# praisechan/Chameleon-RAG-Acceleration

Measured on AMD Instinct MI355X. Metric: queries/sec + recall@10, SIFT1M IVF-PQ (nlist=1024, M=16, nprobe=16), higher is better.
Workload: dtype f32; 1 GPU; IVF1024,PQ16x8 search, d=128, nb=1000000, nprobe=16, k=10, batch=1024 queries per GPU per step; parallelism=single GPU, global_batch=1024, inflight=2, key=nb1000000-d128-IVF1024-PQ16-np16-k10-B1024-w1-single-c200000

## Files before the change

chameleon-rag-acceleration_amd/csrc/ivfpq_index.cpp:

```cpp
#include <hip/hip_runtime.h>

#include <algorithm>
#include <cmath>
#include <cstdio>
#include <cstdlib>
#include <cstring>
#include <memory>
#include <mutex>
#include <stdexcept>
#include <string>
#include <vector>

#include "ivfpq.h"
#include "ivfpq_test.h"
#include "ivfpq_kernels.h"
#include "ivfpq_build.h"
#include "pq_flat.h"

using namespace chivf;

namespace {

thread_local std::string g_err;

// ... 32 lines not shown
  ~DevBuf() { release(); }
};

struct DeviceGuard {
  int prev = -1;
  explicit DeviceGuard(int dev) {
    HIPCHECK(hipGetDevice(&prev));
    if (prev != dev) HIPCHECK(hipSetDevice(dev));
  }
  ~DeviceGuard() {
    int cur = -1;
    if (hipGetDevice(&cur) == hipSuccess && cur != prev && prev >= 0) (void)hipSetDevice(prev);
  }
};

uint64_t splitmix(uint64_t* s) {
  uint64_t z = (*s += 0x9E3779B97F4A7C15ull);
  z = (z ^ (z >> 30)) * 0xBF58476D1CE4E5B9ull;
  z = (z ^ (z >> 27)) * 0x94D049BB133111EBull;
  return z ^ (z >> 31);
}

std::vector<int64_t> rand_perm_prefix(int64_t n, int64_t k, uint64_t seed) {
  std::vector<int64_t> p(n), out(k);
  for (int64_t i = 0; i < n; i++) p[i] = i;
  uint64_t s = seed;
  for (int64_t i = 0; i < k; i++) {
    int64_t j = i + (int64_t)(splitmix(&s) % (uint64_t)(n - i));
    std::swap(p[i], p[j]);
    out[i] = p[i];
  }
  return out;
}

void renorm_rows(float* x, int64_t n, int d) {
  for (int64_t i = 0; i < n; i++) {
    float* xi = x + i * d;
    float nr = 0.f;
    for (int t = 0; t < d; t++) nr += xi[t] * xi[t];
    if (nr > 0.f) {
      const float inv = (float)(1.0 / (double)sqrtf(nr));
      for (int t = 0; t < d; t++) xi[t] *= inv;
    }
  }
}

void kmeans_update(const float* x, int64_t n, int d, int k, const int64_t* assign, float* cent) {
  std::vector<double> sum((size_t)k * d, 0.0);
  std::vector<int64_t> cnt(k, 0);
  for (int64_t i = 0; i < n; i++) {
    const int64_t c = assign[i];
    cnt[c]++;
    double* s = &sum[(size_t)c * d];
    const float* xi = x + i * d;
    for (int t = 0; t < d; t++) s[t] += (double)xi[t];
  }
  for (int c = 0; c < k; c++)
    if (cnt[c] > 0)
      for (int t = 0; t < d; t++) cent[(size_t)c * d + t] = (float)(sum[(size_t)c * d + t] / (double)cnt[c]);
  const float eps = 1.0f / 1024.0f;
  for (int c = 0; c < k; c++) {
    if (cnt[c] != 0) continue;
    int big = 0;
    for (int j = 1; j < k; j++)
      if (cnt[j] > cnt[big]) big = j;
    for (int t = 0; t < d; t++) {
      const float v = cent[(size_t)big * d + t];
      if (t % 2 == 0) {
        cent[(size_t)c * d + t] = v * (1.0f + eps);
        cent[(size_t)big * d + t] = v * (1.0f - eps);
      } else {
        cent[(size_t)c * d + t] = v * (1.0f - eps);
        cent[(size_t)big * d + t] = v * (1.0f + eps);
      }
    }
    cnt[c] = cnt[big] / 2;
    cnt[big] -= cnt[c];
  }
}

constexpr size_t kChunkBytes = size_t(256) << 20;
constexpr size_t kPartialBytes = size_t(2048) << 20;
constexpr int kSegmentedNlist = 8192;
constexpr int kInflightFreeCus = 16;

bool inflight_default() {
  const char* e = std::getenv("IVFPQ_INFLIGHT");
  return e && e[0] == '1';
}

}

struct ivfpq_index {
  int d = 0, nlist = 0, M = 0, nbits = 8, ksub = 256, metric = IVFPQ_METRIC_L2, device = 0;
  int nprobe = 1;
  int list_lo = 0, list_hi = 0;
  bool trained = false;
  std::vector<float> centroids, codebook;
  std::vector<std::vector<uint8_t>> lcodes;
  std::vector<std::vector<int64_t>> lids;
  int64_t ntotal = 0;
  int64_t next_id = 0;

  DevBuf d_cent, d_centT, d_cnorm, d_cb, d_T1, d_codes, d_ids, d_off, d_order;
  bool dirty = true;
  hipStream_t stream = nullptr;
  DevBuf w_x, w_xn, w_D, w_I, w_lno, w_codes, w_cent, w_cn;
  DevBuf h_D, h_I, h_Iq, h_Dq;
  DevBuf q_lists, q_ids, q_codes, a_off;
  int64_t q_n = 0, q_kept = 0, q_cap = 0;
  int64_t img_n = 0;
  bool host_stale = false;
  struct PreT3 {
    DevBuf buf;
    int64_t n = 0;
    uint64_t seq = 0;
    uint64_t freed_seq = 0;
    hipEvent_t ready = nullptr;
    hipStream_t ready_stream = nullptr;
    hipEvent_t freed = nullptr;
    hipStream_t freed_stream = nullptr;
    bool ready_pending = false, freed_pending = false;
  };
  static constexpr int kPreT3 = 3;
  PreT3 pre[kPreT3];
  uint64_t pre_seq = 0;
  struct Work {
    DevBuf w_dist, w_lists, w_dis0, w_T3, w_cand;
    DevBuf w_qn;
    DevBuf p_cnt, p_bucket, p_recs, p_hdr, p_part, p_N, p_pd0, p_done, p_tau, p_qmask, p_evlog;
    uint32_t epoch = 0;
    hipEvent_t done = nullptr;
    hipStream_t done_stream = nullptr;
    bool done_pending = false;
    uint64_t last_use = 0;
  };
  static constexpr int kSlots = 3;
  Work work[kSlots];
  int slot = 0;
  uint64_t uses = 0;
  bool inflight = inflight_default();
  int fault_inj = 0;
  std::vector<uint64_t> tau_seed;
  std::mutex mu;

  Work& W() { return work[slot]; }
  void begin_slot(hipStream_t s) {
    int pick = -1;
    for (int i = 0; i < kSlots && pick < 0; i++)
      if (work[i].done_pending && work[i].done_stream == s) pick = i;
    if (pick < 0) {
      pick = 0;
      for (int i = 1; i < kSlots; i++)
        if (work[i].last_use < work[pick].last_use) pick = i;
    }
    slot = pick;
    Work& w = work[slot];
    w.last_use = ++uses;
    if (w.done_pending && w.done_stream != s) {
      HIPCHECK(hipEventSynchronize(w.done));
      w.done_pending = false;
    }
    if (!inflight) order_after_all(s);
  }
  void order_after_all(hipStream_t s) {
    for (auto& w : work)
      if (w.done_pending && w.done_stream != s) HIPCHECK(hipStreamWaitEvent(s, w.done, 0));
  }
  void mark_done(hipStream_t s) {
    Work& w = W();
    HIPCHECK(hipEventRecord(w.done, s));
    w.done_stream = s;
    w.done_pending = true;
  }
  void quiesce() {
    for (auto& w : work) {
      if (w.done_pending) HIPCHECK(hipEventSynchronize(w.done));
      w.done_pending = false;
    }
  }

  ListPlan make_plan(int64_t nq, int np, int k, hipStream_t s, bool leave_free = false) {
    const int nloc = std::max(list_hi - list_lo, 1);
    Work& w = W();
    const int G = list_scan_group(M, k);
    ListPlan pl;
    pl.cap = (int)nq;
    pl.max_items = list_scan_max_items(nq * np, nloc, G);
    pl.grid = scan_lists_grid(M, k, leave_free ? kInflightFreeCus : 0);
    if (!w.p_cnt.p || w.p_cnt.bytes < sizeof(int32_t) * 2 * nloc) {
      w.p_cnt.ensure(sizeof(int32_t) * 2 * nloc);
      HIPCHECK(hipMemsetAsync(w.p_cnt.p, 0, w.p_cnt.bytes, s));
    }
    w.p_bucket.ensure(sizeof(int2) * 2 * (size_t)nloc * nq);
    w.p_recs.ensure(sizeof(int32_t) * 16 * (size_t)pl.max_items);
    if (!w.p_hdr.p) {
      w.p_hdr.ensure(sizeof(int32_t) * 16);
      HIPCHECK(hipMemsetAsync(w.p_hdr.p, 0, w.p_hdr.bytes, s));
    }
    pl.ks = part_stride(k);
    w.p_part.ensure(sizeof(uint4) * nq * np * 4 * pl.ks);
    w.p_N.ensure(sizeof(uint2) * nq * np * 4);
    w.p_pd0.ensure(sizeof(float) * nq * np);
    if (!w.p_evlog.p) {
      w.p_evlog.ensure(sizeof(uint32_t) * 8 * kEvLog);
      HIPCHECK(hipMemsetAsync(w.p_evlog.p, 0, w.p_evlog.bytes, s));
    }
    if (!w.p_done.p || w.p_done.bytes < sizeof(int32_t) * nq) {
      w.p_done.ensure(sizeof(int32_t) * nq);
      HIPCHECK(hipMemsetAsync(w.p_done.p, 0, w.p_done.bytes, s));
    }
    if (!w.p_tau.p || w.p_tau.bytes < sizeof(uint64_t) * nq) {
      w.p_tau.ensure(sizeof(uint64_t) * nq);
      HIPCHECK(hipMemsetAsync(w.p_tau.p, 0xff, w.p_tau.bytes, s));
    }
    if (++w.epoch >= 0xFFFFFFF0u) {
      if (w.done_pending) HIPCHECK(hipEventSynchronize(w.done));
      HIPCHECK(hipMemsetAsync(w.p_tau.p, 0xff, w.p_tau.bytes, s));
      w.epoch = 1;
    }
    if (!tau_seed.empty()) {
      std::vector<uint64_t> seed;
      seed.swap(tau_seed);
      require((int64_t)seed.size() == nq, "seeded bounds: one per query of the next batch (single-chunk searches)");
      for (auto& v : seed) v = ((uint64_t)(~w.epoch) << 32) | (uint32_t)v;
      HIPCHECK(hipMemcpyAsync(w.p_tau.p, seed.data(), sizeof(uint64_t) * nq, hipMemcpyHostToDevice, s));
      HIPCHECK(hipStreamSynchronize(s));
    }
    pl.qmw = (np + 63) / 64;
    w.p_qmask.ensure(sizeof(uint64_t) * nq * pl.qmw);
    pl.cnt = w.p_cnt.as<int32_t>();
    pl.bucket = w.p_bucket.as<int2>();
    pl.recs = w.p_recs.as<int32_t>();
    pl.hdr = w.p_hdr.as<int32_t>();
    pl.part = w.p_part.as<uint4>();
    pl.partN = w.p_N.as<uint2>();
    pl.pd0 = w.p_pd0.as<float>();
    pl.evlog = w.p_evlog.as<uint32_t>();
    pl.fault = fault_inj;
    pl.qdone = w.p_done.as<int32_t>();
    pl.tauq = w.p_tau.as<uint64_t>();
    pl.epoch = w.epoch;
    pl.err = w.p_hdr.as<int32_t>() + 15;
    pl.qmask = w.p_qmask.as<uint64_t>();
    pl.order = d_order.p ? d_order.as<int32_t>() : nullptr;
    pl.fused = scan_fused_plan(nloc, pl.max_items, M) ? 1 : 0;
    return pl;
  }

  enum Stage { ST_COARSE = 0, ST_TABLES = 1, ST_SCAN = 2, ST_LISTS = 3, ST_N = 4 };
  int timing = 0;
  struct Mark {
    int stage;
    hipEvent_t a, b;
  };
  std::vector<Mark> marks;
  std::vector<hipEvent_t> ev_pool;

  hipEvent_t take_event() {
    if (!ev_pool.empty()) {
      hipEvent_t e = ev_pool.back();
      ev_pool.pop_back();
      return e;
    }
    hipEvent_t e;
    HIPCHECK(hipEventCreate(&e));
    return e;
  }
  int mark_begin(int stage, hipStream_t s, bool record = true) {
    if (!timing || (timing == 2 && stage != ST_LISTS)) return -1;
    Mark m{stage, take_event(), take_event()};
    if (record) HIPCHECK(hipEventRecord(m.a, s));
    marks.push_back(m);
    return (int)marks.size() - 1;
  }
  void mark_end(int idx, hipStream_t s) {
    if (idx >= 0) HIPCHECK(hipEventRecord(marks[idx].b, s));
  }
  void collect_timing(double* ms, int64_t* cnt) {
    for (int i = 0; i < ST_N; i++) {
      ms[i] = 0.0;
      cnt[i] = 0;
    }
    for (auto& m : marks) {
      HIPCHECK(hipEventSynchronize(m.b));
      float t = 0.f;
      HIPCHECK(hipEventElapsedTime(&t, m.a, m.b));
      ms[m.stage] += t;
      cnt[m.stage] += 1;
      ev_pool.push_back(m.a);
      ev_pool.push_back(m.b);
    }
    marks.clear();
  }

  ~ivfpq_index() {
    for (auto& m : marks) {
      (void)hipEventDestroy(m.a);
      (void)hipEventDestroy(m.b);
    }
    for (auto e : ev_pool) (void)hipEventDestroy(e);
    for (auto& w : work)
      if (w.done) (void)hipEventDestroy(w.done);
    for (auto& p : pre) {
      if (p.ready) (void)hipEventDestroy(p.ready);
      if (p.freed) (void)hipEventDestroy(p.freed);
    }
    if (stream) (void)hipStreamDestroy(stream);
  }

  void init_stream() {
    if (!stream) HIPCHECK(hipStreamCreateWithFlags(&stream, hipStreamNonBlocking));
    for (auto& w : work)
      if (!w.done) HIPCHECK(hipEventCreateWithFlags(&w.done, hipEventDisableTiming));
    for (auto& p : pre) {
      if (!p.ready) HIPCHECK(hipEventCreateWithFlags(&p.ready, hipEventDisableTiming));
      if (!p.freed) HIPCHECK(hipEventCreateWithFlags(&p.freed, hipEventDisableTiming));
    }
  }

  void assign_top1(const float* x_host, int64_t n, int dd, const float* dc, const float* dcn, int nc,
                   int64_t* assign_host, const float* x_dev = nullptr, bool ip_assign = false) {
    const int64_t rows = std::max<int64_t>(1, std::min<int64_t>(n, kChunkBytes / ((size_t)nc * 4)));
    w_xn.ensure(sizeof(float) * rows);
    W().w_dist.ensure(sizeof(float) * rows * nc);
    w_D.ensure(sizeof(float) * rows);
    w_I.ensure(sizeof(int64_t) * rows);
    if (!x_dev) w_x.ensure(sizeof(float) * rows * dd);
    for (int64_t r0 = 0; r0 < n; r0 += rows) {
// ... 1580 lines not shown
```

chameleon-rag-acceleration_amd/csrc/ivfpq_kernels.h:

```cpp
#pragma once
#include <hip/hip_runtime.h>
#include <stdint.h>

namespace chivf {

constexpr int kMaxK = 1024;
constexpr int64_t kSentinelId = INT64_MAX;

void launch_row_norms(const float* x, int64_t n, int d, float* out, hipStream_t s);

void launch_l2_dist(const float* x, const float* xn, int64_t nx, const float* c, const float* cn, int nc, int d,
                    float* out, hipStream_t s, bool ip = false);

void launch_select_rows(const float* dist, int64_t nrows, int ncols, int n, float* out_val, int64_t* out_col,
                        hipStream_t s, bool neg = false);

struct ListPlan;

bool coarse_tiled_ok(int d, int64_t nq);
void launch_coarse_keys(const float* x, int64_t nq, int d, const float* centT, const float* cn, int nlist,
                        float* keys, hipStream_t s, bool ip, float* T3out = nullptr, const float* cb = nullptr,
                        int M = 0, float* xn_buf = nullptr, const float* xt = nullptr, int64_t nt = 0,
                        bool hoist = false);
void launch_coarse_select(const float* keys, int64_t nq, int nlist, int nprobe, float* out_dis, int64_t* out_list,
                          hipStream_t s, bool ip, const ListPlan* plan = nullptr, const int64_t* list_off = nullptr,
                          int lo = 0, int hi = 0, const float* x = nullptr, const float* cent = nullptr, int d = 0);

int coarse_segments(int64_t nq, int nlist, int d);
void launch_coarse_segmented(const float* x, int64_t nq, int d, const float* centT, const float* cn, int nlist,
                             int nprobe, uint64_t* cand, float* out_dis, int64_t* out_list, hipStream_t s, bool ip,
                             const ListPlan* plan = nullptr, const int64_t* list_off = nullptr, int lo = 0, int hi = 0,
                             const float* cent = nullptr);

void launch_linear_transform(const float* x, int64_t n, int d_in, const float* AT, const float* b, int d_out, float* y,
                             hipStream_t s);

void launch_ip_table(const float* x, int64_t n, int d, const float* codebook, int M, int ksub, float* out,
                     hipStream_t s);

void launch_precompute_T1(const float* cent, int nlist, int d, const float* codebook, int M, int ksub, float* T1,
                          hipStream_t s);

void launch_pq_encode(const float* x, int64_t n, int d, const float* cent, const int64_t* list_no,
                      const float* codebook, int M, int ksub, uint8_t* codes, hipStream_t s);

inline int part_stride(int k) { return k; }

constexpr int kHdrLog = 12;
constexpr int kHdrStale = 13;
constexpr int kHdrRepair = 14;
constexpr int kEvLog = 64;

struct ListPlan {
  int32_t* cnt;
  int2* bucket;
  int cap;
  int32_t* recs;
  int32_t* hdr;
  int max_items;
  uint4* part;
  uint2* partN;
  float* pd0;
  int32_t* qdone;
  uint64_t* tauq;
  uint32_t epoch;
  int32_t* err;
  uint64_t* qmask;
  int qmw = 1;
  uint32_t* evlog;
  int fault = 0;
  int grid;
  const int32_t* order = nullptr;
  int fused = 0;
  int ks = 0;
};

struct ScanArgs {
  const float* T1;
  const float* T3;
  const uint8_t* codes;
  const int64_t* ids;
  const int64_t* list_off;
  int64_t n_codes;
  const int64_t* probe_list;
  int64_t nq;
  int nprobe;
  int k;
  int M;
  int ip;
  int list_lo, list_hi;
  float* outD;
  int64_t* outI;
};

void launch_plan_count(const int64_t* lists, const float* Dq, const float* x, const float* cent, int64_t nq, int d,
                       int nprobe, const int64_t* list_off, int lo, int hi, bool ip, bool dedup, int k,
                       const ListPlan& pl, hipStream_t s);
void launch_plan_items(const ListPlan& pl, const int64_t* list_off, int lo, int hi, int G, hipStream_t s);
bool scan_fused_plan(int nloc, int max_items, int M);

int list_scan_group(int M, int k);
int list_scan_max_items(int64_t npairs, int nloc, int G);
int scan_lists_grid(int M, int k, int free_cus = 0);
bool scan_supported_M(int M);
void launch_scan_lists(const ScanArgs& a, const ListPlan& plan, hipStream_t s, hipEvent_t* ev_lists = nullptr);

void launch_merge_topk(int S, int64_t n, int k, const float* Din, const int64_t* Iin, float* Dout, int64_t* Iout,
                       hipStream_t s, bool ip = false);

}
```

chameleon-rag-acceleration_amd/csrc/ivfpq_kernels.hip:

```cpp
#include <float.h>
#include <stdint.h>

#include <algorithm>
#include <type_traits>

#include <hip/hip_runtime.h>

#include "ivfpq_kernels.h"
#include "ivfpq_diag.h"

namespace chivf {

namespace {

constexpr float kInf = __builtin_huge_valf();

enum { K_IP = 0, K_L2 = 1, K_NORM = 2 };

template <int KIND, class FX, class FY>
__device__ __forceinline__ float tree(FX fx, FY fy, int d) {
  float a8[8] = {0.f, 0.f, 0.f, 0.f, 0.f, 0.f, 0.f, 0.f};
  int i = 0;
  for (; i + 8 <= d; i += 8) {
#pragma unroll
// ... 2111 lines not shown
#pragma unroll
                for (int g = 0; g < G; g++) {
                  if ((mk[g] >> lane) & 1) {
                    const int sl = g * QG + qn[g] + __popcll(mk[g] & lanemask_lt);
                    qd[wave][sl] = dis[j][g];
                    qi[wave][sl] = i;
                  }
                  qn[g] += __popcll(mk[g]);
                  DIAG_ONLY(d_push += __popcll(mk[g]);)
                }
                if (loose) {
                  stop = j + 1;
                  want = true;
                  go = false;
                }
              }
            }
          }
        }
        if (stop >= tn) {
          pend = want;
          break;
        }
        drain();
        t = stop;
      }
      bool queued = false;
#pragma unroll
      for (int g = 0; g < G; g++) queued = queued || qn[g] > 0;
      DIAG_ONLY(const uint64_t tc0 = __builtin_amdgcn_s_memtime(); d_admit += tc0 - tb0;)
      if (pend || (last_sb && queued)) {
        drain();
      }
      DIAG_ONLY(asm volatile("" ::"v"(ROWK ? rk : tk[0].p[0])); d_fdrain += __builtin_amdgcn_s_memtime() - tc0;)
    }
    DIAG(2, __builtin_amdgcn_s_memtime());
    DIAG(4, n);
    DIAG(5, it.cnt | (it.kind << 8));
    DIAG(6, d_gather);
    DIAG(7, d_push | (d_drain << 32));
    DIAG(8, d_loose);
    DIAG(9, d_admit);
    DIAG(10, d_fdrain);

    if constexpr (ROWK) {
      const int rg = lane >> 4, re = lane & 15;
      int pr = it.pair[0];
#pragma unroll
      for (int g = 1; g < G; g++) pr = rg == g ? it.pair[g] : pr;
      const int64_t slot = (int64_t)pr * 4 + wave;
      if (rg < it.cnt && re < k && !(pl.fault > 0 && slot % pl.fault == 1)) {
        const bool empty = rk == kKcNone;
        pl.part[slot * pl.ks + re] =
            part_rec(empty ? FLT_MAX : kc_key(rk), part_tag(pl.epoch, slot) | xcc_tag(), empty ? -1 : it.beg + (int64_t)(uint32_t)rk);
      }
    } else {
#pragma unroll
      for (int g = 0; g < G; g++) {
        if (g >= it.cnt) continue;
        write_partial<R>(pl, tk[g], (int64_t)it.pair[g] * 4 + wave, k, it.beg, lane);
      }
    }
    if (nxt >= 0) {
      unpack(nrec);
      if constexpr (kEarly) issue();
    }
    DIAG(3, __builtin_amdgcn_s_memtime());
    it_no++;
    cur = nxt;
  }
}

#ifndef SCAN_LEAN
#define SCAN_LEAN 1
#endif
#ifndef SCAN_PREFETCH
#define SCAN_PREFETCH 0
#endif
constexpr bool kScanLean = SCAN_LEAN != 0;
constexpr bool kScanPrefetch = SCAN_PREFETCH != 0;
#ifndef SCAN_LEAN_JB
#define SCAN_LEAN_JB 6
#endif
constexpr int kLeanJB = SCAN_LEAN_JB;

__device__ __forceinline__ uint64_t pack_kc_bits(uint32_t b, uint32_t pos) {
  b = b == 0x80000000u ? 0u : b;
  const uint32_t o = (int32_t)b >= 0 ? (b ^ 0x80000000u) : ~b;
  return ((uint64_t)o << 32) | pos;
}
__device__ __forceinline__ uint64_t row_shr1_u64(uint64_t v) {
  const uint32_t lo = (uint32_t)__builtin_amdgcn_update_dpp((int)(uint32_t)v, (int)(uint32_t)v, 0x111, 0xf, 0xf, false);
  const uint32_t hi =
      (uint32_t)__builtin_amdgcn_update_dpp((int)(uint32_t)(v >> 32), (int)(uint32_t)(v >> 32), 0x111, 0xf, 0xf, false);
  return ((uint64_t)hi << 32) | lo;
}

template <int M, int JB>
__global__ __launch_bounds__(256, 2) void k_scan_lean(ScanArgs a, ListPlan pl) {
  constexpr int G = 4;
  constexpr int LUTN = M * 256;
  constexpr int NV = LUTN / 4 / 256;
  static_assert(NV <= 4 && JB % 2 == 0, "lean scan: M <= 16");
  __shared__ __attribute__((aligned(16))) float4 lut[LUTN];
  __shared__ int s_next;
  __shared__ int32_t s_wb[G];
  __shared__ int s_ws[8];
  __shared__ uint16_t s_ex[2][kFusedPlanLists + 1];
  __shared__ uint16_t s_ord[kFusedPlanLists];

  const int tid = threadIdx.x;
  const int lane = tid & 63;
  const int wave = __builtin_amdgcn_readfirstlane(tid >> 6);
  const int k = a.k;
  const int ip = a.ip;
  const int nloc = a.list_hi - a.list_lo;
  const float inv_np = 1.0f / (float)a.nprobe;
  const int rg = lane >> 4, re = lane & 15;
  const int2 nn = fused_plan_prefix(pl, nloc, G, s_ex[0], s_ex[1], s_ord, s_ws);
  const int n_items0 = nn.x, n_items = nn.x + nn.y;

  Item<G> it;
  auto unpack = [&](const Rec& rc) __attribute__((always_inline)) {
    const int rv = rc.raw;
    it.l = rc.l;
    it.kind = rc.kind;
    it.cnt = min(G, min(__builtin_amdgcn_readlane(rv, 1), pl.cap) - rc.t * G);
    it.n = __builtin_amdgcn_readlane(rv, 2) - __builtin_amdgcn_readlane(rv, 3);
    it.beg = (int64_t)(((uint64_t)(uint32_t)__builtin_amdgcn_readlane(rv, 4) << 32) |
                       (uint32_t)__builtin_amdgcn_readlane(rv, 3));
#pragma unroll
    for (int g = 0; g < G; g++) {
      it.pair[g] = __builtin_amdgcn_readlane(rv, 5 + g);
      it.d0[g] = __int_as_float(__builtin_amdgcn_readlane(rv, 9 + g));
    }
    bool bad = false;
#pragma unroll
    for (int g = 0; g < G; g++) bad = bad || (g < it.cnt && (unsigned)it.pair[g] >= (unsigned)(a.nq * a.nprobe));
    if (bad) {
      if (lane == 0) atomicAdd(pl.err, 1);
      it.cnt = 0;
#pragma unroll
      for (int g = 0; g < G; g++) it.pair[g] = 0;
    }
#pragma unroll
    for (int g = 0; g < G; g++) it.q[g] = div_small((g < it.cnt ? it.pair[g] : it.pair[0]), a.nprobe, inv_np);
  };
  auto fetch_rec = [&](int idx) __attribute__((always_inline)) {
    return fused_record(a, pl, nloc, idx, n_items0, s_ex[0], s_ex[1], s_ord, G, lane);
  };

  if (tid == 0) {
    const int t = atomicAdd(pl.hdr + 2, 1);
    s_next = t < n_items ? t : -1;
  }
  __syncthreads();
  int cur = s_next;
  if (cur >= 0) unpack(fetch_rec(cur));
  CodeWords<M> cw[JB];
  uint64_t tw[G];
  float4 b1[NV], b3[NV][G];
  auto prefetch_t3 = [&](const int (&q)[G]) __attribute__((always_inline)) {
#pragma unroll
    for (int g = 0; g < G; g++) tw[g] = tau_load(pl, q[g]);
#pragma unroll
    for (int e = 0; e < NV; e++) {
      const int v = e * 256 + tid;
#pragma unroll
      for (int g = 0; g < G; g++) b3[e][g] = reinterpret_cast<const float4*>(a.T3 + (int64_t)q[g] * LUTN)[v];
    }
  };
  auto load_t1 = [&](int l, int q0) __attribute__((always_inline)) {
    const float4* T1l = reinterpret_cast<const float4*>(ip ? a.T3 + (int64_t)q0 * LUTN : a.T1 + (int64_t)l * LUTN);
#pragma unroll
    for (int e = 0; e < NV; e++) b1[e] = T1l[e * 256 + tid];
  };
  if (kScanPrefetch && cur >= 0) prefetch_t3(it.q);
  int it_no = 0;
  (void)it_no;
  while (cur >= 0) {
    __syncthreads();
    DIAG(0, __builtin_amdgcn_s_memtime());
    int tnext;
    if (tid == 0) tnext = atomicAdd(pl.hdr + 2, 1);
    if (!kScanPrefetch) prefetch_t3(it.q);
    load_t1(it.l, it.q[0]);
    const int n = it.n;
    const uint8_t* lc = a.codes + it.beg * M;
#pragma unroll
    for (int j = 0; j < JB; j++) {
      const int i = j * 256 + wave * 64 + lane;
      cw[j].load(lc + (int64_t)(i < n ? i : 0) * M);
    }
#pragma unroll
    for (int e = 0; e < NV; e++) {
      const int v = e * 256 + tid;
#pragma unroll
      for (int c = 0; c < 4; c++) {
        float4 o;
#pragma unroll
        for (int g = 0; g < G; g++) {
          const float x3 = comp(b3[e][g], c);
          setc(o, g, ip ? -x3 : __builtin_fmaf(x3, -2.0f, comp(b1[e], c)));
        }
        lut[4 * v + c] = o;
      }
    }
    if (tid == 0) s_next = tnext < n_items ? tnext : -1;
    if (tid < G) s_wb[tid] = f2ord(kInf);
    __syncthreads();
    DIAG(1, __builtin_amdgcn_s_memtime());
    const int nxt = s_next;
    const Rec nrec = fetch_rec(nxt >= 0 ? nxt : cur);
    const int cnt = it.cnt;
    int pr = it.pair[0];
#pragma unroll
    for (int g = 1; g < G; g++) pr = rg == g ? it.pair[g] : pr;
    const int64_t slot = (int64_t)pr * 4 + wave;
    const bool st = rg < cnt && re < k && !(pl.fault > 0 && slot % pl.fault == 1);
    const int64_t beg = it.beg;
    int qix[G];
    float bound[G];
    bool loose = false;
    uint64_t rtp[G];
#pragma unroll
    for (int g = 0; g < G; g++) {
      qix[g] = it.q[g];
      bound[g] = g < cnt ? ord2f(tau_decode(pl, tw[g])) : -kInf;
      loose = loose || bound[g] == kInf;
      rtp[g] = kKcNone;
    }
    uint64_t rk = kKcNone;
    uint32_t pub = 0;
    DIAG_ONLY(uint64_t d_gather = 0, d_bounds = 0, d_admit = 0, n_ins = 0;)

    uint32_t ins = 0;
    auto insert = [&](int g, uint64_t v) __attribute__((always_inline)) {
      if (!(v < rtp[g])) return;
      const uint64_t lt = __builtin_amdgcn_ballot_w64(rk < v);
      const int p = __popcll((lt >> (16 * g)) & 0xFFFFull);
      const uint64_t sh = row_shr1_u64(rk);
      rk = rg == g ? (re > p ? sh : (re == p ? v : rk)) : rk;
      ins |= 1u << g;
      DIAG_ONLY(n_ins++;)
    };
    auto refresh = [&]() __attribute__((always_inline)) {
#pragma unroll
      for (int g = 0; g < G; g++) {
        if ((ins >> g) & 1u) {
          rtp[g] = readlane_u64(rk, 16 * g + k - 1);
          if (rtp[g] != kKcNone) bound[g] = fminf(bound[g], kc_key(rtp[g]));
        }
      }
      pub |= ins;
      ins = 0;
    };
    auto publish = [&]() __attribute__((always_inline)) {
#pragma unroll
      for (int g = 0; g < G; g++) {
        if (((pub >> g) & 1u) && rtp[g] != kKcNone && lane == 0) {
          atomicMin(&s_wb[g], f2ord(kc_key(rtp[g])));
          tau_lower(pl, qix[g], f2ord(kc_key(rtp[g])));
        }
      }
      pub = 0;
    };

    DIAG(11, __builtin_amdgcn_s_memtime());
    for (int sb = 0; sb < n; sb += 256 * JB) {
      DIAG_ONLY(const uint64_t tg0 = __builtin_amdgcn_s_memtime();)
      const int tn = max(0, min(JB, (n - sb - 64 * wave + 255) >> 8));
      const bool last_sb = sb + 256 * JB >= n;
      float dis[JB][G];
#pragma unroll
      for (int jd = 0; jd < JB / 2; jd++) {
        if (2 * jd + 1 < tn) {
          CodeWords<M> cc[2] = {cw[2 * jd], cw[2 * jd + 1]};
#pragma unroll
          for (int h = 0; h < 2; h++)
#pragma unroll
            for (int v = 0; v < M / 4; v++) asm volatile("" : "+v"(cc[h].w[v]));
#pragma unroll
          for (int h = 0; h < 2; h++)
#pragma unroll
            for (int g = 0; g < G; g++) dis[2 * jd + h][g] = it.d0[g];
#pragma unroll
          for (int m = 0; m < M; m++) {
#pragma unroll
            for (int h = 0; h < 2; h++) {
              const float4 v = lut[m * 256 + cc[h].byte(m)];
#pragma unroll
              for (int g = 0; g < G; g++) dis[2 * jd + h][g] = dis[2 * jd + h][g] + comp(v, g);
            }
          }
        } else if (2 * jd < tn) {
          CodeWords<M> cc = cw[2 * jd];
#pragma unroll
          for (int v = 0; v < M / 4; v++) asm volatile("" : "+v"(cc.w[v]));
#pragma unroll
          for (int g = 0; g < G; g++) dis[2 * jd][g] = it.d0[g];
#pragma unroll
          for (int m = 0; m < M; m++) {
            const float4 v = lut[m * 256 + cc.byte(m)];
#pragma unroll
            for (int g = 0; g < G; g++) dis[2 * jd][g] = dis[2 * jd][g] + comp(v, g);
          }
        }
      }
      DIAG_ONLY(asm volatile("" ::"v"(dis[0][0]), "v"(dis[JB - 1][G - 1])); const uint64_t tg1 = __builtin_amdgcn_s_memtime(); d_gather += tg1 - tg0;)
      if (!last_sb) {
#pragma unroll
        for (int j = 0; j < JB; j++) {
          const int i = sb + 256 * JB + j * 256 + wave * 64 + lane;
          cw[j].load(lc + (int64_t)(i < n ? i : 0) * M);
        }
      }
      if (kScanPrefetch && last_sb && nxt >= 0) {
        unpack(nrec);
        prefetch_t3(it.q);
      }
      if (loose) {
#pragma unroll
        for (int g = 0; g < G; g++) {
          if (bound[g] != kInf) continue;
          float mn = kInf;
#pragma unroll
          for (int j = 0; j < JB; j++)
            if (j < tn && sb + j * 256 + wave * 64 + lane < n) mn = fminf(mn, dis[j][g]);
          const float T = wave_kth_smallest(mn, k, lane);
          if (T < kInf && lane == 0) {
            atomicMin(&s_wb[g], f2ord(T));
            tau_lower(pl, qix[g], f2ord(T));
          }
        }
      }
      loose = false;
#pragma unroll
      for (int g = 0; g < G; g++) {
        if (g < cnt) bound[g] = fminf(bound[g], ord2f(__builtin_amdgcn_readfirstlane(s_wb[g])));
        loose = loose || bound[g] == kInf;
      }
      DIAG_ONLY(const uint64_t tb1 = __builtin_amdgcn_s_memtime(); d_bounds += tb1 - tg1;)
#pragma unroll
      for (int j = 0; j < JB; j++) {
        if (j < tn) {
          const int i0 = sb + j * 256 + wave * 64;
          const bool valid = i0 + lane < n;
          bool c = false;
#pragma unroll
          for (int g = 0; g < G; g++) c = c || dis[j][g] <= bound[g];
          if (__builtin_amdgcn_ballot_w64(valid && c) == 0) continue;
#pragma unroll
          for (int g = 0; g < G; g++) {
            uint64_t mk = __builtin_amdgcn_ballot_w64(valid && dis[j][g] <= bound[g]);
            while (mk) {
              const int src = (int)__builtin_ctzll(mk);
              mk &= mk - 1;
              const uint32_t b = (uint32_t)__builtin_amdgcn_readlane((int)__float_as_uint(dis[j][g]), src);
              insert(g, pack_kc_bits(b, (uint32_t)(i0 + src)));
            }
          }
        }
      }
      refresh();
      DIAG_ONLY(d_admit += __builtin_amdgcn_s_memtime() - tb1;)
      if (!last_sb) publish();
    }
    DIAG(2, __builtin_amdgcn_s_memtime());
    DIAG(4, n);
    DIAG(5, it.cnt | (it.kind << 8));
    DIAG(6, d_gather);
    DIAG(7, n_ins);
    DIAG(8, d_bounds);
    DIAG(9, d_admit);
    DIAG(10, 0);
    if (!kScanPrefetch && nxt >= 0) unpack(nrec);
    publish();
    if (st) {
      const bool empty = rk == kKcNone;
      pl.part[slot * pl.ks + re] =
          part_rec(empty ? FLT_MAX : kc_key(rk), part_tag(pl.epoch, slot) | xcc_tag(), empty ? -1 : beg + (int64_t)(uint32_t)rk);
    }
    DIAG(3, __builtin_amdgcn_s_memtime());
    DIAG_ONLY(it_no++;)
    cur = nxt;
  }
}

constexpr int kSegQ = 128;
__global__ __launch_bounds__(256) void k_coarse_segtop(const float* __restrict__ x, int64_t nq, int d,
                                                       const float* __restrict__ centT, int ldc,
                                                       const float* __restrict__ cn, int nlist, int ip, int seg,
                                                       int nseg, int nprobe, uint64_t* __restrict__ cand) {
  extern __shared__ __attribute__((aligned(16))) float g_lds[];
  const int tid = threadIdx.x;
  const int lane = tid & 63;
  const int wave = tid >> 6;
  const int64_t q0 = (int64_t)(blockIdx.x / nseg) * GQ;
  const int sg = blockIdx.x % nseg;
  const int cb = sg * seg, ce = min(nlist, cb + seg);
  const int dk = (d + 63) & ~63;
  float* xs = g_lds;
  float* xn = xs + dk * GQ;
  float* kt = xn + GQ + GQ * 8;
  uint64_t* cq = reinterpret_cast<uint64_t*>(kt + GQ * GC);
  coarse_stage_queries(xs, xn, x, q0, nq, d, dk, tid);
  const int i16 = lane & 15, k4 = lane >> 4;
  const uint64_t lt = (1ull << lane) - 1;
  PackedTopK<1> tk[4];
  int qn[4];
#pragma unroll
  for (int u = 0; u < 4; u++) {
    tk[u].init(nprobe);
    qn[u] = 0;
  }
  auto drain = [&](int u) __attribute__((always_inline)) {
    uint64_t* qv = cq + (wave * 4 + u) * kSegQ;
    for (int b = 0; b < qn[u]; b += 64) {
      uint64_t c = b + lane < qn[u] ? qv[b + lane] : kKcNone;
      c = c < tk[u].tp ? c : kKcNone;
      if (__builtin_amdgcn_ballot_w64(c != kKcNone)) kc_bulk_merge(tk[u], c, lane);
    }
    qn[u] = 0;
  };
  for (int t0 = cb; t0 < ce; t0 += GC) {
    f4 acc[NTL];
    coarse_key_tile(acc, xs, GQ, 0, centT, ldc, nlist, d, dk, t0 + wave * 32, lane);
    __syncthreads();
#pragma unroll
    for (int t = 0; t < NTL; t++) {
      const int c = t0 + wave * 32 + t * 16 + i16;
      const float cnv = ip ? 0.f : cn[min(c, nlist - 1)];
#pragma unroll
      for (int r = 0; r < 4; r++) {
        const int i = k4 * 4 + r;
        kt[i * GC + wave * 32 + t * 16 + i16] = coarse_key(acc[t][r], xn[i], cnv, ip);
      }
    }
    __syncthreads();
#pragma unroll
    for (int u = 0; u < 4; u++) {
      const int i = wave * 4 + u;
#pragma unroll
      for (int h = 0; h < GC / 64; h++) {
        const int c = t0 + h * 64 + lane;
        const uint64_t p = c < ce ? pack_kc(kt[i * GC + h * 64 + lane], c) : kKcNone;
        const bool pass = p < tk[u].tp;
        const uint64_t mk = __builtin_amdgcn_ballot_w64(pass);
        if (!mk) continue;
        const int cnt = (int)__popcll(mk);
        if (qn[u] + cnt > kSegQ) drain(u);
        if (pass) cq[i * kSegQ + qn[u] + (int)__popcll(mk & lt)] = p;
        qn[u] += cnt;
      }
    }
  }
#pragma unroll
  for (int u = 0; u < 4; u++) {
    drain(u);
    const int64_t q = q0 + wave * 4 + u;
    if (q < nq && lane < nprobe) cand[(q * nseg + sg) * nprobe + lane] = tk[u].p[0];
  }
}
// ... 984 lines not shown
  if (n <= 0) return;
  const int dsub = d / M;
  const dim3 grid((unsigned)n);
  if (d > 2048 || (M * ksub) % 16 != 0) return;
  if (ksub == 256 && n >= GQ) {
    const dim3 tg((unsigned)(nblocks(n, GQ) * (unsigned)M));
    switch (dsub) {
      case 2: hipLaunchKernelGGL(k_ip_tiles<2>, tg, dim3(256), 0, s, x, n, d, cb, M, out); return;
      case 4: hipLaunchKernelGGL(k_ip_tiles<4>, tg, dim3(256), 0, s, x, n, d, cb, M, out); return;
      case 8: hipLaunchKernelGGL(k_ip_tiles<8>, tg, dim3(256), 0, s, x, n, d, cb, M, out); return;
      case 12: hipLaunchKernelGGL(k_ip_tiles<12>, tg, dim3(256), 0, s, x, n, d, cb, M, out); return;
      case 16: hipLaunchKernelGGL(k_ip_tiles<16>, tg, dim3(256), 0, s, x, n, d, cb, M, out); return;
      default: break;
    }
  }
  switch (dsub) {
    case 2: hipLaunchKernelGGL(k_ip_table<2>, grid, dim3(256), 0, s, x, n, d, cb, M, ksub, out); break;
    case 4: hipLaunchKernelGGL(k_ip_table<4>, grid, dim3(256), 0, s, x, n, d, cb, M, ksub, out); break;
    case 8: hipLaunchKernelGGL(k_ip_table<8>, grid, dim3(256), 0, s, x, n, d, cb, M, ksub, out); break;
    case 12: hipLaunchKernelGGL(k_ip_table<12>, grid, dim3(256), 0, s, x, n, d, cb, M, ksub, out); break;
    case 16: hipLaunchKernelGGL(k_ip_table<16>, grid, dim3(256), 0, s, x, n, d, cb, M, ksub, out); break;
    default: hipLaunchKernelGGL(k_ip_table<0>, grid, dim3(256), 0, s, x, n, d, cb, M, ksub, out); break;
  }
}

void launch_precompute_T1(const float* cent, int nlist, int d, const float* cb, int M, int ksub, float* T1,
                          hipStream_t s) {
  hipLaunchKernelGGL(k_precompute_T1, dim3(nblocks((int64_t)nlist * M * ksub, 256)), dim3(256), 0, s, cent, nlist,
                     d, cb, M, ksub, T1);
}

void launch_pq_encode(const float* x, int64_t n, int d, const float* cent, const int64_t* list_no,
                      const float* cb, int M, int ksub, uint8_t* codes, hipStream_t s) {
  if (n <= 0) return;
  hipLaunchKernelGGL(k_pq_encode, dim3(nblocks(n * M, 256)), dim3(256), 0, s, x, n, d, cent, list_no, cb, M, ksub,
                     codes);
}

void launch_plan_count(const int64_t* lists, const float* Dq, const float* x, const float* cent, int64_t nq, int d,
                       int nprobe, const int64_t* list_off, int lo, int hi, bool ip, bool dedup, int k,
                       const ListPlan& pl, hipStream_t s) {
  if (nq <= 0) return;
  hipLaunchKernelGGL(k_plan_count, dim3(nblocks(nq, 4)), dim3(256), 0, s, lists, Dq, x, cent, nq, d, nprobe,
                     list_off, lo, hi, ip ? 1 : 0, dedup ? 1 : 0, k, pl);
}

bool scan_fused_plan(int nloc, int max_items, int M) {
  return nloc <= kFusedPlanLists && max_items < 65536 && M > 0;
}

void launch_plan_items(const ListPlan& pl, const int64_t* list_off, int lo, int hi, int G, hipStream_t s) {
  if (pl.fused) return;
  const int nloc = hi - lo;
  if (nloc <= kPlanSmall)
    hipLaunchKernelGGL(k_plan_items_small, dim3(std::max(1u, nblocks(pl.max_items, PLAN_T))), dim3(PLAN_T), 0, s, pl,
                       list_off, lo, nloc, G);
  else
    hipLaunchKernelGGL(k_plan_items_big, dim3(std::max(1u, nblocks(nloc, PLAN_T))), dim3(PLAN_T), 0, s, pl, list_off,
                       lo, nloc, G);
}

bool scan_supported_M(int M) { return M == 8 || M == 16 || M == 32 || M == 48 || M == 64; }
constexpr int scan_group(int M, int R) {
  return (M * 1024 * 4 <= 65536 && 4 * R <= 8 && !(R >= 2 && M <= 16)) ? 4
         : (M * 1024 * 2 <= 65536 && 2 * R <= 8)                      ? 2
                                                                      : 1;
}
int list_scan_group(int M, int k) {
  const int R = rows_for(k);
  switch (R) {
    case 1: return scan_group(M, 1);
    case 2: return scan_group(M, 2);
    case 4: return scan_group(M, 4);
    case 8: return scan_group(M, 8);
    default: return scan_group(M, 16);
  }
}

int list_scan_max_items(int64_t npairs, int nloc, int G) {
  const int64_t v = (npairs + G - 1) / G + std::min<int64_t>(2 * (int64_t)nloc, npairs) + 8;
  return (int)v;
}

int scan_lists_grid(int M, int k, int free_cus) {
  static int cus = 0;
  if (!cus) {
    int dev = 0, n = 256;
    if (hipGetDevice(&dev) == hipSuccess) (void)hipDeviceGetAttribute(&n, hipDeviceAttributeMultiprocessorCount, dev);
    cus = n;
  }
  const int lds = M * 256 * 4 * list_scan_group(M, k) + 4 * QCAP * 8 + 6 * kFusedPlanLists + 96;
  const int per_cu = std::max(1, std::min(3, 160 * 1024 / lds));
#ifdef SCAN_GRID_QUARTERS
  if (per_cu == 2) return std::max(8, (SCAN_GRID_QUARTERS * cus / 4 + 7) / 8 * 8);
#endif
  static int env_free = -2;
  if (env_free == -2) {
    const char* e = getenv("IVFPQ_SCAN_FREE_CUS");
    env_free = e ? std::max(0, atoi(e)) : -1;
  }
  if (env_free >= 0) free_cus = env_free;
  free_cus = std::max(0, std::min(free_cus, cus / 2));
  return std::max(8, (per_cu * (cus - free_cus) + 7) / 8 * 8);
}

int device_cus() {
  static int cus = 0;
  if (!cus) {
    int dev = 0, n = 256;
    if (hipGetDevice(&dev) == hipSuccess) (void)hipDeviceGetAttribute(&n, hipDeviceAttributeMultiprocessorCount, dev);
    cus = n;
  }
  return cus;
}

template <int M, int R>
static void launch_lists_MR(const ScanArgs& a, const ListPlan& pl, hipStream_t s, hipEvent_t* ev) {
  constexpr int G = scan_group(M, R);
  constexpr int JB = M <= 16 ? 6 : 4;
  if (ev) (void)hipEventRecord(ev[0], s);
  if constexpr (G == 4 && R == 1) {
    if (a.k <= 16 && pl.fused && kScanLean && M <= 16) {
      hipLaunchKernelGGL((k_scan_lean<M, kLeanJB>), dim3((unsigned)pl.grid), dim3(256), 0, s, a, pl);
    } else if (a.k <= 16) {
      hipLaunchKernelGGL((k_scan_lists<M, G, R, JB, true>), dim3((unsigned)pl.grid), dim3(256), 0, s, a, pl);
    } else {
      hipLaunchKernelGGL((k_scan_lists<M, G, R, JB>), dim3((unsigned)pl.grid), dim3(256), 0, s, a, pl);
    }
  } else {
    hipLaunchKernelGGL((k_scan_lists<M, G, R, JB>), dim3((unsigned)pl.grid), dim3(256), 0, s, a, pl);
  }
  if (ev) (void)hipEventRecord(ev[1], s);
  if (R >= 2 && a.nprobe <= 64) {
    if (4 * a.nprobe * pl.ks <= kRadixU * 256)
      hipLaunchKernelGGL(k_merge_radix, dim3((unsigned)a.nq), dim3(256), 0, s, a, pl);
    else
      hipLaunchKernelGGL(k_merge_big, dim3((unsigned)a.nq), dim3(64), 0, s, a, pl);
  }
  hipLaunchKernelGGL(k_merge_probes<R>, dim3(nblocks(a.nq, 4)), dim3(256), 0, s, a, pl);
#ifdef DIAG_TWICE
  if (R == 1) hipLaunchKernelGGL(k_merge_probes<R>, dim3(nblocks(a.nq, 4)), dim3(256), 0, s, a, pl);
#endif
}

template <int M>
static void launch_lists_M(const ScanArgs& a, const ListPlan& pl, hipStream_t s, hipEvent_t* ev) {
  switch (rows_for(a.k)) {
    case 1: launch_lists_MR<M, 1>(a, pl, s, ev); break;
    case 2: launch_lists_MR<M, 2>(a, pl, s, ev); break;
    case 4: launch_lists_MR<M, 4>(a, pl, s, ev); break;
    case 8: launch_lists_MR<M, 8>(a, pl, s, ev); break;
    default: launch_lists_MR<M, 16>(a, pl, s, ev); break;
  }
}

void launch_scan_lists(const ScanArgs& a, const ListPlan& pl, hipStream_t s, hipEvent_t* ev_lists) {
  if (a.nq <= 0) return;
  switch (a.M) {
    case 8: launch_lists_M<8>(a, pl, s, ev_lists); break;
    case 16: launch_lists_M<16>(a, pl, s, ev_lists); break;
    case 32: launch_lists_M<32>(a, pl, s, ev_lists); break;
    case 48: launch_lists_M<48>(a, pl, s, ev_lists); break;
    case 64: launch_lists_M<64>(a, pl, s, ev_lists); break;
    default: break;
  }
}

void launch_merge_topk(int S, int64_t n, int k, const float* Din, const int64_t* Iin, float* Dout, int64_t* Iout,
                       hipStream_t s, bool ip) {
  if (n <= 0) return;
  hipLaunchKernelGGL(k_merge_topk, dim3((unsigned)n), dim3(256), 0, s, S, n, k, Din, Iin, Dout, Iout, ip ? 1 : 0);
}

}

#if defined(DIAG_STAMPS) || defined(DIAG_CSTAMPS)
extern "C" int ivfpq_diag_stamps(void* out, size_t bytes) {
  if (hipMemcpyFromSymbol(out, HIP_SYMBOL(chivf::g_diag), bytes) != hipSuccess) return -1;
  static uint64_t zeros[chivf::kDiagWG * chivf::kDiagItems * chivf::kDiagSlots];
  return hipMemcpyToSymbol(HIP_SYMBOL(chivf::g_diag), zeros, sizeof(zeros)) == hipSuccess ? 0 : -1;
}
#endif
```

Baseline: 10.10 million queries/s.

## Split lean scan LUT into two halves to raise occupancy for M=16

For M=16 the lean list-scan kernel now holds only half of the per-list lookup table in LDS at a time. It builds and gathers over each half in two passes with extra barriers, and drops T3 prefetch, so three workgroups can fit per CU instead of two. The scan grid is now sized from the occupancy API for the lean kernel, and the in-flight mode reserves more free CUs (96) when the split kernel is used. The gain is more concurrent waves; the cost is rebuilding LUT halves per superblock, which adds global loads and syncs.

```diff
diff --git a/chameleon-rag-acceleration_amd/csrc/ivfpq_index.cpp b/chameleon-rag-acceleration_amd/csrc/ivfpq_index.cpp
--- a/chameleon-rag-acceleration_amd/csrc/ivfpq_index.cpp
+++ b/chameleon-rag-acceleration_amd/csrc/ivfpq_index.cpp
@@ -138,8 +138,6 @@
 constexpr size_t kChunkBytes = size_t(256) << 20;
 constexpr size_t kPartialBytes = size_t(2048) << 20;
 constexpr int kSegmentedNlist = 8192;
-constexpr int kInflightFreeCus = 16;
-
 bool inflight_default() {
   const char* e = std::getenv("IVFPQ_INFLIGHT");
   return e && e[0] == '1';
@@ -243,7 +241,6 @@
     ListPlan pl;
     pl.cap = (int)nq;
     pl.max_items = list_scan_max_items(nq * np, nloc, G);
-    pl.grid = scan_lists_grid(M, k, leave_free ? kInflightFreeCus : 0);
     if (!w.p_cnt.p || w.p_cnt.bytes < sizeof(int32_t) * 2 * nloc) {
       w.p_cnt.ensure(sizeof(int32_t) * 2 * nloc);
       HIPCHECK(hipMemsetAsync(w.p_cnt.p, 0, w.p_cnt.bytes, s));
@@ -301,6 +298,7 @@
     pl.qmask = w.p_qmask.as<uint64_t>();
     pl.order = d_order.p ? d_order.as<int32_t>() : nullptr;
     pl.fused = scan_fused_plan(nloc, pl.max_items, M) ? 1 : 0;
+    pl.grid = scan_lists_grid(M, k, pl.fused != 0, leave_free ? scan_inflight_free_cus(M, k, pl.fused != 0) : 0);
     return pl;
   }
 
diff --git a/chameleon-rag-acceleration_amd/csrc/ivfpq_kernels.h b/chameleon-rag-acceleration_amd/csrc/ivfpq_kernels.h
--- a/chameleon-rag-acceleration_amd/csrc/ivfpq_kernels.h
+++ b/chameleon-rag-acceleration_amd/csrc/ivfpq_kernels.h
@@ -101,7 +101,8 @@
 
 int list_scan_group(int M, int k);
 int list_scan_max_items(int64_t npairs, int nloc, int G);
-int scan_lists_grid(int M, int k, int free_cus = 0);
+int scan_lists_grid(int M, int k, bool fused, int free_cus = 0);
+int scan_inflight_free_cus(int M, int k, bool fused);
 bool scan_supported_M(int M);
 void launch_scan_lists(const ScanArgs& a, const ListPlan& plan, hipStream_t s, hipEvent_t* ev_lists = nullptr);
 
diff --git a/chameleon-rag-acceleration_amd/csrc/ivfpq_kernels.hip b/chameleon-rag-acceleration_amd/csrc/ivfpq_kernels.hip
--- a/chameleon-rag-acceleration_amd/csrc/ivfpq_kernels.hip
+++ b/chameleon-rag-acceleration_amd/csrc/ivfpq_kernels.hip
@@ -2217,7 +2217,15 @@
 #ifndef SCAN_LEAN_JB
 #define SCAN_LEAN_JB 6
 #endif
-constexpr int kLeanJB = SCAN_LEAN_JB;
+#ifndef SCAN_LEAN_SPLIT
+#define SCAN_LEAN_SPLIT 1
+#endif
+#ifndef SCAN_LEAN_SPLIT_JB
+#define SCAN_LEAN_SPLIT_JB 6
+#endif
+constexpr bool lean_split(int M) { return SCAN_LEAN_SPLIT != 0 && M == 16; }
+constexpr int lean_jb(int M) { return lean_split(M) ? SCAN_LEAN_SPLIT_JB : SCAN_LEAN_JB; }
+constexpr int kInflightFreeCus = 16, kInflightFreeCusSplit = 96;
 
 __device__ __forceinline__ uint64_t pack_kc_bits(uint32_t b, uint32_t pos) {
   b = b == 0x80000000u ? 0u : b;
@@ -2231,13 +2239,18 @@
   return ((uint64_t)hi << 32) | lo;
 }
 
-template <int M, int JB>
-__global__ __launch_bounds__(256, 2) void k_scan_lean(ScanArgs a, ListPlan pl) {
+template <int M, int JB, bool SPLIT>
+__global__ __launch_bounds__(256, SPLIT ? 3 : 2) void k_scan_lean(ScanArgs a, ListPlan pl) {
   constexpr int G = 4;
   constexpr int LUTN = M * 256;
   constexpr int NV = LUTN / 4 / 256;
   static_assert(NV <= 4 && JB % 2 == 0, "lean scan: M <= 16");
-  __shared__ __attribute__((aligned(16))) float4 lut[LUTN];
+  constexpr int NP = SPLIT ? 2 : 1;
+  constexpr int NH = NV / NP;
+  constexpr int MH = M / NP;
+  static_assert(NV % NP == 0 && (M / 4) % NP == 0, "lean scan: a pass is whole float4 rows and whole code words");
+  constexpr bool kPre = kScanPrefetch && !SPLIT;
+  __shared__ __attribute__((aligned(16))) float4 lut[LUTN / NP];
   __shared__ int s_next;
   __shared__ int32_t s_wb[G];
   __shared__ int s_ws[8];
@@ -2253,7 +2266,11 @@
   const float inv_np = 1.0f / (float)a.nprobe;
   const int rg = lane >> 4, re = lane & 15;
   const int2 nn = fused_plan_prefix(pl, nloc, G, s_ex[0], s_ex[1], s_ord, s_ws);
-  const int n_items0 = nn.x, n_items = nn.x + nn.y;
+  const int n_items0 = nn.x, n_items = SPLIT ? __builtin_amdgcn_readfirstlane(nn.x + nn.y) : nn.x + nn.y;
+  auto opq = [&](int v) __attribute__((always_inline)) {
+    if constexpr (SPLIT) asm volatile("" : "+v"(v));
+    return v;
+  };
 
   Item<G> it;
   auto unpack = [&](const Rec& rc) __attribute__((always_inline)) {
@@ -2282,7 +2299,7 @@
     for (int g = 0; g < G; g++) it.q[g] = div_small((g < it.cnt ? it.pair[g] : it.pair[0]), a.nprobe, inv_np);
   };
   auto fetch_rec = [&](int idx) __attribute__((always_inline)) {
-    return fused_record(a, pl, nloc, idx, n_items0, s_ex[0], s_ex[1], s_ord, G, lane);
+    return fused_record(a, pl, nloc, idx, n_items0, s_ex[0], s_ex[1], s_ord, G, opq(lane));
   };
 
   if (tid == 0) {
@@ -2294,23 +2311,56 @@
   if (cur >= 0) unpack(fetch_rec(cur));
   CodeWords<M> cw[JB];
   uint64_t tw[G];
-  float4 b1[NV], b3[NV][G];
+  float4 b1[NH], b3[NH][G];
   auto prefetch_t3 = [&](const int (&q)[G]) __attribute__((always_inline)) {
-#pragma unroll
-    for (int g = 0; g < G; g++) tw[g] = tau_load(pl, q[g]);
-#pragma unroll
-    for (int e = 0; e < NV; e++) {
-      const int v = e * 256 + tid;
-#pragma unroll
-      for (int g = 0; g < G; g++) b3[e][g] = reinterpret_cast<const float4*>(a.T3 + (int64_t)q[g] * LUTN)[v];
+    if constexpr (!SPLIT) {
+#pragma unroll
+      for (int g = 0; g < G; g++) tw[g] = tau_load(pl, q[g]);
+#pragma unroll
+      for (int e = 0; e < NV; e++) {
+        const int v = e * 256 + tid;
+#pragma unroll
+        for (int g = 0; g < G; g++) b3[e][g] = reinterpret_cast<const float4*>(a.T3 + (int64_t)q[g] * LUTN)[v];
+      }
     }
   };
   auto load_t1 = [&](int l, int q0) __attribute__((always_inline)) {
-    const float4* T1l = reinterpret_cast<const float4*>(ip ? a.T3 + (int64_t)q0 * LUTN : a.T1 + (int64_t)l * LUTN);
-#pragma unroll
-    for (int e = 0; e < NV; e++) b1[e] = T1l[e * 256 + tid];
+    if constexpr (!SPLIT) {
+      const float4* T1l = reinterpret_cast<const float4*>(ip ? a.T3 + (int64_t)q0 * LUTN : a.T1 + (int64_t)l * LUTN);
+#pragma unroll
+      for (int e = 0; e < NV; e++) b1[e] = T1l[e * 256 + tid];
+    }
   };
-  if (kScanPrefetch && cur >= 0) prefetch_t3(it.q);
+  auto load_rows = [&](int hf) __attribute__((always_inline)) {
+    const int tid = opq(threadIdx.x);
+    const float4* T1l =
+        reinterpret_cast<const float4*>(ip ? a.T3 + (int64_t)it.q[0] * LUTN : a.T1 + (int64_t)it.l * LUTN);
+#pragma unroll
+    for (int e = 0; e < NH; e++) {
+      const int v = (hf * NH + e) * 256 + tid;
+#pragma unroll
+      for (int g = 0; g < G; g++) b3[e][g] = reinterpret_cast<const float4*>(a.T3 + (int64_t)it.q[g] * LUTN)[v];
+      b1[e] = T1l[v];
+    }
+  };
+  auto store_rows = [&]() __attribute__((always_inline)) {
+    const int tid = opq(threadIdx.x);
+#pragma unroll
+    for (int e = 0; e < NH; e++) {
+      const int v = e * 256 + tid;
+#pragma unroll
+      for (int c = 0; c < 4; c++) {
+        float4 o;
+#pragma unroll
+        for (int g = 0; g < G; g++) {
+          const float x3 = comp(b3[e][g], c);
+          setc(o, g, ip ? -x3 : __builtin_fmaf(x3, -2.0f, comp(b1[e], c)));
+        }
+        lut[4 * v + c] = o;
+      }
+    }
+  };
+  if (kPre && cur >= 0) prefetch_t3(it.q);
   int it_no = 0;
   (void)it_no;
   while (cur >= 0) {
@@ -2318,8 +2368,14 @@
     DIAG(0, __builtin_amdgcn_s_memtime());
     int tnext;
     if (tid == 0) tnext = atomicAdd(pl.hdr + 2, 1);
-    if (!kScanPrefetch) prefetch_t3(it.q);
-    load_t1(it.l, it.q[0]);
+    if constexpr (SPLIT) {
+#pragma unroll
+      for (int g = 0; g < G; g++) tw[g] = tau_load(pl, it.q[g]);
+      load_rows(0);
+    } else {
+      if (!kPre) prefetch_t3(it.q);
+      load_t1(it.l, it.q[0]);
+    }
     const int n = it.n;
     const uint8_t* lc = a.codes + it.beg * M;
 #pragma unroll
@@ -2327,22 +2383,9 @@
       const int i = j * 256 + wave * 64 + lane;
       cw[j].load(lc + (int64_t)(i < n ? i : 0) * M);
     }
-#pragma unroll
-    for (int e = 0; e < NV; e++) {
-      const int v = e * 256 + tid;
-#pragma unroll
-      for (int c = 0; c < 4; c++) {
-        float4 o;
-#pragma unroll
-        for (int g = 0; g < G; g++) {
-          const float x3 = comp(b3[e][g], c);
-          setc(o, g, ip ? -x3 : __builtin_fmaf(x3, -2.0f, comp(b1[e], c)));
-        }
-        lut[4 * v + c] = o;
-      }
-    }
+    store_rows();
     if (tid == 0) s_next = tnext < n_items ? tnext : -1;
-    if (tid < G) s_wb[tid] = f2ord(kInf);
+    if (const int t = opq(tid); t < G) s_wb[t] = f2ord(kInf);
     __syncthreads();
     DIAG(1, __builtin_amdgcn_s_memtime());
     const int nxt = s_next;
@@ -2407,40 +2450,68 @@
       const int tn = max(0, min(JB, (n - sb - 64 * wave + 255) >> 8));
       const bool last_sb = sb + 256 * JB >= n;
       float dis[JB][G];
-#pragma unroll
-      for (int jd = 0; jd < JB / 2; jd++) {
-        if (2 * jd + 1 < tn) {
-          CodeWords<M> cc[2] = {cw[2 * jd], cw[2 * jd + 1]};
-#pragma unroll
-          for (int h = 0; h < 2; h++)
-#pragma unroll
-            for (int v = 0; v < M / 4; v++) asm volatile("" : "+v"(cc[h].w[v]));
-#pragma unroll
-          for (int h = 0; h < 2; h++)
-#pragma unroll
-            for (int g = 0; g < G; g++) dis[2 * jd + h][g] = it.d0[g];
-#pragma unroll
-          for (int m = 0; m < M; m++) {
-#pragma unroll
-            for (int h = 0; h < 2; h++) {
-              const float4 v = lut[m * 256 + cc[h].byte(m)];
-#pragma unroll
-              for (int g = 0; g < G; g++) dis[2 * jd + h][g] = dis[2 * jd + h][g] + comp(v, g);
+      auto gather = [&](int hf) __attribute__((always_inline)) {
+#pragma unroll
+        for (int jd = 0; jd < JB / 2; jd++) {
+          if (2 * jd + 1 < tn) {
+            uint32_t cc[2][MH / 4];
+#pragma unroll
+            for (int h = 0; h < 2; h++)
+#pragma unroll
+              for (int v = 0; v < MH / 4; v++) {
+                cc[h][v] = cw[2 * jd + h].w[hf * (MH / 4) + v];
+                asm volatile("" : "+v"(cc[h][v]));
+              }
+            if (hf == 0) {
+#pragma unroll
+              for (int h = 0; h < 2; h++)
+#pragma unroll
+                for (int g = 0; g < G; g++) dis[2 * jd + h][g] = it.d0[g];
+            }
+#pragma unroll
+            for (int m = 0; m < MH; m++) {
+#pragma unroll
+              for (int h = 0; h < 2; h++) {
+                const float4 v = lut[m * 256 + ((cc[h][m >> 2] >> ((m & 3) * 8)) & 0xffu)];
+#pragma unroll
+                for (int g = 0; g < G; g++) dis[2 * jd + h][g] = dis[2 * jd + h][g] + comp(v, g);
+              }
+            }
+          } else if (2 * jd < tn) {
+            uint32_t cc[MH / 4];
+#pragma unroll
+            for (int v = 0; v < MH / 4; v++) {
+              cc[v] = cw[2 * jd].w[hf * (MH / 4) + v];
+              asm volatile("" : "+v"(cc[v]));
+            }
+            if (hf == 0) {
+#pragma unroll
+              for (int g = 0; g < G; g++) dis[2 * jd][g] = it.d0[g];
+            }
+#pragma unroll
+            for (int m = 0; m < MH; m++) {
+              const float4 v = lut[m * 256 + ((cc[m >> 2] >> ((m & 3) * 8)) & 0xffu)];
+#pragma unroll
+              for (int g = 0; g < G; g++) dis[2 * jd][g] = dis[2 * jd][g] + comp(v, g);
             }
           }
-        } else if (2 * jd < tn) {
-          CodeWords<M> cc = cw[2 * jd];
-#pragma unroll
-          for (int v = 0; v < M / 4; v++) asm volatile("" : "+v"(cc.w[v]));
-#pragma unroll
-          for (int g = 0; g < G; g++) dis[2 * jd][g] = it.d0[g];
-#pragma unroll
-          for (int m = 0; m < M; m++) {
-            const float4 v = lut[m * 256 + cc.byte(m)];
-#pragma unroll
-            for (int g = 0; g < G; g++) dis[2 * jd][g] = dis[2 * jd][g] + comp(v, g);
-          }
         }
+      };
+      if constexpr (SPLIT) {
+        if (sb > 0) {
+          load_rows(0);
+          __syncthreads();
+          store_rows();
+          __syncthreads();
+        }
+        gather(0);
+        load_rows(1);
+        __syncthreads();
+        store_rows();
+        __syncthreads();
+        gather(1);
+      } else {
+        gather(0);
       }
       DIAG_ONLY(asm volatile("" ::"v"(dis[0][0]), "v"(dis[JB - 1][G - 1])); const uint64_t tg1 = __builtin_amdgcn_s_memtime(); d_gather += tg1 - tg0;)
       if (!last_sb) {
@@ -2450,7 +2521,7 @@
           cw[j].load(lc + (int64_t)(i < n ? i : 0) * M);
         }
       }
-      if (kScanPrefetch && last_sb && nxt >= 0) {
+      if (kPre && last_sb && nxt >= 0) {
         unpack(nrec);
         prefetch_t3(it.q);
       }
@@ -2509,11 +2580,11 @@
     DIAG(8, d_bounds);
     DIAG(9, d_admit);
     DIAG(10, 0);
-    if (!kScanPrefetch && nxt >= 0) unpack(nrec);
+    if (!kPre && nxt >= 0) unpack(nrec);
     publish();
     if (st) {
       const bool empty = rk == kKcNone;
-      pl.part[slot * pl.ks + re] =
+      pl.part[slot * pl.ks + opq(re)] =
           part_rec(empty ? FLT_MAX : kc_key(rk), part_tag(pl.epoch, slot) | xcc_tag(), empty ? -1 : beg + (int64_t)(uint32_t)rk);
     }
     DIAG(3, __builtin_amdgcn_s_memtime());
@@ -3664,7 +3735,28 @@
   return (int)v;
 }
 
-int scan_lists_grid(int M, int k, int free_cus) {
+static bool scan_uses_lean(int M, int k, bool fused) {
+  return kScanLean && fused && k <= 16 && (M == 8 || M == 16) && list_scan_group(M, k) == 4;
+}
+
+static int lean_wgs_per_cu(int M) {
+  static int cache[2] = {0, 0};
+  int& c = cache[M == 16 ? 1 : 0];
+  if (!c) {
+    int n = 0;
+    const hipError_t e =
+        M == 16 ? hipOccupancyMaxActiveBlocksPerMultiprocessor(&n, k_scan_lean<16, lean_jb(16), lean_split(16)>, 256, 0)
+                : hipOccupancyMaxActiveBlocksPerMultiprocessor(&n, k_scan_lean<8, lean_jb(8), lean_split(8)>, 256, 0);
+    c = e == hipSuccess && n > 0 ? n : (lean_split(M) ? 3 : 2);
+  }
+  return c;
+}
+
+int scan_inflight_free_cus(int M, int k, bool fused) {
+  return scan_uses_lean(M, k, fused) && lean_split(M) ? kInflightFreeCusSplit : kInflightFreeCus;
+}
+
+int scan_lists_grid(int M, int k, bool fused, int free_cus) {
   static int cus = 0;
   if (!cus) {
     int dev = 0, n = 256;
@@ -3672,7 +3764,7 @@
     cus = n;
   }
   const int lds = M * 256 * 4 * list_scan_group(M, k) + 4 * QCAP * 8 + 6 * kFusedPlanLists + 96;
-  const int per_cu = std::max(1, std::min(3, 160 * 1024 / lds));
+  const int per_cu = scan_uses_lean(M, k, fused) ? lean_wgs_per_cu(M) : std::max(1, std::min(3, 160 * 1024 / lds));
 #ifdef SCAN_GRID_QUARTERS
   if (per_cu == 2) return std::max(8, (SCAN_GRID_QUARTERS * cus / 4 + 7) / 8 * 8);
 #endif
@@ -3701,9 +3793,9 @@
   constexpr int G = scan_group(M, R);
   constexpr int JB = M <= 16 ? 6 : 4;
   if (ev) (void)hipEventRecord(ev[0], s);
-  if constexpr (G == 4 && R == 1) {
-    if (a.k <= 16 && pl.fused && kScanLean && M <= 16) {
-      hipLaunchKernelGGL((k_scan_lean<M, kLeanJB>), dim3((unsigned)pl.grid), dim3(256), 0, s, a, pl);
+  if constexpr (G == 4 && R == 1 && M <= 16) {
+    if (scan_uses_lean(M, a.k, pl.fused != 0)) {
+      hipLaunchKernelGGL((k_scan_lean<M, lean_jb(M), lean_split(M)>), dim3((unsigned)pl.grid), dim3(256), 0, s, a, pl);
     } else if (a.k <= 16) {
       hipLaunchKernelGGL((k_scan_lists<M, G, R, JB, true>), dim3((unsigned)pl.grid), dim3(256), 0, s, a, pl);
     } else {
```

Measured after the change: 10.25 million queries/s, median of 6. +1.5%, better.
